# Aedelon/MASt3R-SLAM

Measured on AMD Instinct MI355X. Metric: keyframe-pairs/sec (512x512 two-view infer+match+GN), higher is better.
Workload: dtype fp16

## Files before the change

### mast3r-slam_amd/csrc/conv_tail.hip

```cpp
#include "gemm_common.h"

using namespace m3gemm;

namespace {

constexpr int kThreads = 512;
constexpr int TH = 16, TW = 32;
constexpr int HH = TH + 2, HW = TW + 2;
constexpr int kHaloPix = HH * HW;
constexpr int kHaloBytes = kHaloPix * 128;
constexpr int kWStage = 128 * 128;
constexpr int PH = 11, PW = 19;
constexpr int kPatchBytes = (PH * PW * 128 + 1023) / 1024 * 1024;
constexpr int kLdsBytes = kHaloBytes + 2 * kWStage + kPatchBytes;

struct TailArgs {
    const bf16_t *X;
    const bf16_t *Wc;
    const float *bias;
    const bf16_t *W4;
    const float *b4;
    float *pts, *conf;
    bf16_t *Y;
    const bf16_t *R;
    int cout, relu_in;
    const bf16_t *zero16;
    int B, H, W, IH, IW;
    const bf16_t *Wc2, *W42;
    const float *bias2, *b42;
};

enum { EP_PLAIN = 0 , EP_TAIL = 1 , EP_RELU = 2 ,
       EP_ADD = 3  };

template <int DT, bool UPS, int CIN, int EP>
__global__ void __launch_bounds__(kThreads, 2)
k_conv_tail(const TailArgs ain) {
    constexpr bool TAIL = EP == EP_TAIL;
    static_assert(CIN % 64 == 0 && (TAIL ? CIN == 128 : true), "64-channel steps; the fused tail is the 128-channel head.2");
    constexpr int NQ = CIN / 64;
    TailArgs a = ain;
    if (blockIdx.y == 1) {
        a.Wc = ain.Wc2; a.W4 = ain.W42; a.bias = ain.bias2; a.b4 = ain.b42;
        a.X = ain.X + (size_t)ain.B * ain.IH * ain.IW * CIN;
        if (TAIL) {
            a.pts = ain.pts + (size_t)ain.B * ain.H * ain.W * 3;
            a.conf = ain.conf + (size_t)ain.B * ain.H * ain.W;
        } else {
            a.Y = ain.Y + (size_t)ain.B * ain.H * ain.W * ain.cout;
            if (EP == EP_ADD) a.R = ain.R + (size_t)ain.B * ain.H * ain.W * ain.cout;
        }
    }
    if (!TAIL) {
        const int z = blockIdx.z;
        a.Wc += (size_t)z * 128 * 9 * CIN;
        if (a.bias) a.bias += z * 128;
        a.Y += z * 128;
        if (EP == EP_ADD) a.R += z * 128;
    }
    extern __shared__ __attribute__((aligned(16))) unsigned char lds[];
    unsigned char *halo = lds, *wst = lds + kHaloBytes, *patch = lds + kHaloBytes + 2 * kWStage;
    const int tid = threadIdx.x, lane = tid & 63, wave = tid >> 6;
    const int wp = wave >> 1, wc = wave & 1;
    const int tiles_x = (a.W + TW - 1) / TW, tiles_y = a.H / TH;
    const int nwg = tiles_x * tiles_y * a.B;
    const int bid = xcd_remap(blockIdx.x, nwg);
    const int b = bid / (tiles_x * tiles_y), trem = bid - b * tiles_x * tiles_y;
    const int ty = trem / tiles_x, tx = trem - ty * tiles_x;
    const int oy0 = ty * TH, ox0 = tx * TW;
    const bf16_t *img = a.X + (size_t)b * a.IH * a.IW * CIN;

    auto stage_w = [&](int tap, int half, int buf) {
        unsigned char *base = wst + buf * kWStage;
#pragma unroll
        for (int i = 0; i < 2; ++i) {
            const int slot = i * kThreads + tid;
            const int row = slot >> 3, cp = slot & 7;
            const int c = half * 8 + (cp ^ ((row >> 1) & 7));
            glds16(a.Wc + ((size_t)row * 9 + tap) * CIN + c * 8, base + i * (kThreads * 16) + wave * 1024);
        }
    };
    const float sy = UPS && a.H > 1 ? (float)(a.IH - 1) / (float)(a.H - 1) : 0.f;
    const float sx = UPS && a.W > 1 ? (float)(a.IW - 1) / (float)(a.W - 1) : 0.f;
    const int py0 = (int)((float)max(oy0 - 1, 0) * sy), px0 = (int)((float)max(ox0 - 1, 0) * sx);
    auto stage_patch = [&](int half) {
        for (int wi = wave; wi < (PH * PW * 8 + 63) / 64; wi += kThreads / 64) {
            int slot = wi * 64 + lane;
            slot = slot < PH * PW * 8 ? slot : PH * PW * 8 - 1;
            const int pp = slot >> 3, c = slot & 7;
            const int y = min(py0 + pp / PW, a.IH - 1), x = min(px0 + pp % PW, a.IW - 1);
            glds16(img + ((size_t)y * a.IW + x) * CIN + (half * 8 + c) * 8, patch + wi * 1024);
        }
    };
    auto stage_halo_direct = [&](int half) {
        for (int wi = wave; wi < (kHaloPix * 8 + 63) / 64; wi += kThreads / 64) {
            int slot = wi * 64 + lane;
            const bool live = slot < kHaloPix * 8;
            slot = live ? slot : kHaloPix * 8 - 1;
            const int pix = slot >> 3, cp = slot & 7;
            const int hy = pix / HW, hx = pix - hy * HW;
            const int iy = oy0 + hy - 1, ix = ox0 + hx - 1;
            const int c = half * 8 + (cp ^ ((hx >> 1) & 7));
            const bool in = iy >= 0 && iy < a.H && ix >= 0 && ix < a.W;
            const void *src = in ? (const void *)(img + ((size_t)iy * a.IW + ix) * CIN + c * 8) : (const void *)a.zero16;
            if (wi * 64 + 64 <= kHaloPix * 8) glds16(src, halo + wi * 1024);
            else if (live) *reinterpret_cast<uint4 *>(halo + (size_t)slot * 16) = *reinterpret_cast<const uint4 *>(src);
        }
    };
    auto blend_halo = [&]() {
        for (int slot = tid; slot < kHaloPix * 8; slot += kThreads) {
            const int pix = slot >> 3, cp = slot & 7;
            const int hy = pix / HW, hx = pix - hy * HW;
            const int iy = oy0 + hy - 1, ix = ox0 + hx - 1;
            const int c = cp ^ ((hx >> 1) & 7);
            uint4 o = make_uint4(0u, 0u, 0u, 0u);
            if (iy >= 0 && iy < a.H && ix >= 0 && ix < a.W) {
                const float fy = iy * sy, fx = ix * sx;
                int y0 = (int)fy, x0 = (int)fx;
                y0 = min(y0, a.IH - 1); x0 = min(x0, a.IW - 1);
                const int y1 = min(y0 + 1, a.IH - 1), x1 = min(x0 + 1, a.IW - 1);
                const float wy = fy - (float)y0, wx = fx - (float)x0;
                const unsigned char *p = patch + c * 16;
                union U { uint4 q; unsigned w[4]; } q00, q01, q10, q11, r;
                q00.q = *reinterpret_cast<const uint4 *>(p + ((y0 - py0) * PW + (x0 - px0)) * 128);
                q01.q = *reinterpret_cast<const uint4 *>(p + ((y0 - py0) * PW + (x1 - px0)) * 128);
                q10.q = *reinterpret_cast<const uint4 *>(p + ((y1 - py0) * PW + (x0 - px0)) * 128);
                q11.q = *reinterpret_cast<const uint4 *>(p + ((y1 - py0) * PW + (x1 - px0)) * 128);
#pragma unroll
                for (int k = 0; k < 4; ++k) {
                    const float tl = lo16<DT>(q00.w[k]) * (1.f - wx) + lo16<DT>(q01.w[k]) * wx;
                    const float bl = lo16<DT>(q10.w[k]) * (1.f - wx) + lo16<DT>(q11.w[k]) * wx;
                    const float th = hi16<DT>(q00.w[k]) * (1.f - wx) + hi16<DT>(q01.w[k]) * wx;
                    const float bh = hi16<DT>(q10.w[k]) * (1.f - wx) + hi16<DT>(q11.w[k]) * wx;
                    r.w[k] = pack16<DT>(tl * (1.f - wy) + bl * wy, th * (1.f - wy) + bh * wy);
                }
                o = r.q;
            }
            *reinterpret_cast<uint4 *>(halo + (size_t)slot * 16) = o;
        }
    };

    f32x4 acc[8][4];
#pragma unroll
    for (int i = 0; i < 8; ++i)
#pragma unroll
        for (int j = 0; j < 4; ++j) acc[i][j] = f32x4{0.f, 0.f, 0.f, 0.f};
    const int frow = lane & 15, fch = lane >> 4;
    int w_off[4];
#pragma unroll
    for (int j = 0; j < 4; ++j) {
        const int r = wc * 64 + j * 16 + frow;
        w_off[j] = r * 128 + ((fch ^ ((r >> 1) & 7)) << 4);
    }

    const int group = wave >> 2;
    bf16x8 af[8], wf[4];
    const int pix_of_row = (int)((0x3D9F2A40E6C851B7ULL >> (4 * frow)) & 15);
    auto col_offset = [&](int hx) { return hx * 128 + ((fch ^ ((hx >> 1) & 7)) << 4); };
    auto read_frags = [&](int g, int tap, int ks) {
        const int ky = tap / 3, kx = tap - ky * 3;
        const unsigned char *wsrc = wst + (g & 1) * kWStage;
        const int flip = ks << 6;
        const int c0 = col_offset(pix_of_row + kx) ^ flip;
        const int c1 = col_offset(16 + pix_of_row + kx) ^ flip;
        const unsigned char *rowp = halo + (wp * 4 + ky) * (HW * 128);
#pragma unroll
        for (int j = 0; j < 4; ++j) wf[j] = *reinterpret_cast<const bf16x8 *>(wsrc + (w_off[j] ^ flip));
#pragma unroll
        for (int i = 0; i < 8; ++i)
            af[i] = *reinterpret_cast<const bf16x8 *>(rowp + (i >> 1) * (HW * 128) + ((i & 1) ? c1 : c0));
        if (!TAIL && a.relu_in) {
#pragma unroll
            for (int i = 0; i < 8; ++i) af[i] = relu_frag(af[i]);
        }
    };
    auto mfma_all = [&]() {
        __builtin_amdgcn_s_setprio(1);
#pragma unroll
        for (int i = 0; i < 8; ++i)
#pragma unroll
            for (int j = 0; j < 4; ++j) acc[i][j] = mfma16<DT>(wf[j], af[i], acc[i][j]);
        __builtin_amdgcn_s_setprio(0);
    };
    auto phase_end = [&]() {
        __builtin_amdgcn_sched_barrier(0);
        __builtin_amdgcn_s_barrier();
        __builtin_amdgcn_sched_barrier(0);
    };
    auto phase_end_wait = [&]() {
        __builtin_amdgcn_sched_barrier(0);
        asm volatile("s_waitcnt vmcnt(0)" ::: "memory");
        __builtin_amdgcn_s_barrier();
        __builtin_amdgcn_sched_barrier(0);
    };
    auto prefetch_w = [&](int g) { if (g + 1 < 9 * NQ) stage_w((g + 1) % 9, (g + 1) / 9, (g + 1) & 1); };
    auto run_half = [&](int half) {
        if (group == 0) {
#pragma unroll 1
            for (int tap = 0; tap < 9; ++tap) {
                const int g = half * 9 + tap;
                read_frags(g, tap, 0);
                prefetch_w(g);
                asm volatile("s_waitcnt lgkmcnt(0)" ::: "memory");
                phase_end();
                mfma_all();
                phase_end();
                read_frags(g, tap, 1);
                asm volatile("s_waitcnt lgkmcnt(0)" ::: "memory");
                phase_end();
                mfma_all();
                phase_end_wait();
            }
            phase_end();
        } else {
#pragma unroll 1
            for (int tap = 0; tap < 9; ++tap) {
                const int g = half * 9 + tap;
                if (tap > 0) mfma_all();
                phase_end();
                read_frags(g, tap, 0);
                prefetch_w(g);
                asm volatile("s_waitcnt lgkmcnt(0)" ::: "memory");
                phase_end();
                mfma_all();
                phase_end();
                read_frags(g, tap, 1);
                asm volatile("s_waitcnt lgkmcnt(0)" ::: "memory");
                phase_end_wait();
            }
            mfma_all();
            phase_end();
        }
    };

    stage_w(0, 0, 0);
    if (UPS) stage_patch(0); else stage_halo_direct(0);
    asm volatile("s_waitcnt vmcnt(0)" ::: "memory");
    lds_barrier();
#pragma unroll 1
    for (int q = 0; q < NQ; ++q) {
        if (UPS) {
            blend_halo();
            lds_barrier();
            if (q + 1 < NQ) stage_patch(q + 1);
        } else if (q > 0) {
            stage_halo_direct(q);
            asm volatile("s_waitcnt vmcnt(0)" ::: "memory");
            lds_barrier();
        }
        run_half(q);
    }

    if constexpr (EP == EP_ADD) {
        const int r = lane & 15, gq = lane >> 4;
        constexpr int RS = 272;
        unsigned char *wl = halo + wave * (32 * RS);
        float4 bj[4];
#pragma unroll
        for (int j = 0; j < 4; ++j)
            bj[j] = a.bias ? *reinterpret_cast<const float4 *>(a.bias + wc * 64 + j * 16 + gq * 4) : make_float4(0.f, 0.f, 0.f, 0.f);
        auto pix = [&](int pass, int rl, int &oy, int &ox) {
            const int i = pass * 2 + (rl >> 4);
            oy = oy0 + wp * 4 + (i >> 1);
            ox = ox0 + (i & 1) * 16 + (int)((0x3D9F2A40E6C851B7ULL >> (4 * (rl & 15))) & 15);
        };
        uint4 q[2][4];
        auto load_resid = [&](int pass, uint4 (&dst)[4]) {
#pragma unroll
            for (int it = 0; it < 4; ++it) {
                const int c = it * 64 + lane, rl = c >> 3, ch = c & 7;
                int oy, ox;
                pix(pass, rl, oy, ox);
                ox = ox < a.W ? ox : a.W - 1;
                dst[it] = *reinterpret_cast<const uint4 *>(a.R + (((size_t)b * a.H + oy) * a.W + ox) * a.cout + wc * 64 + ch * 8);
            }
        };
        load_resid(0, q[0]);
#pragma unroll
        for (int pass = 0; pass < 4; ++pass) {
            if (pass + 1 < 4) load_resid(pass + 1, q[(pass + 1) & 1]);
#pragma unroll
            for (int ii = 0; ii < 2; ++ii)
#pragma unroll
                for (int j = 0; j < 4; ++j) {
                    const f32x4 v = acc[pass * 2 + ii][j];
                    *reinterpret_cast<float4 *>(wl + (ii * 16 + r) * RS + ((j * 4 + gq) << 4)) =
                        make_float4(v[0] + bj[j].x, v[1] + bj[j].y, v[2] + bj[j].z, v[3] + bj[j].w);
                }
            asm volatile("s_waitcnt lgkmcnt(0)" ::: "memory");
#pragma unroll
            for (int it = 0; it < 4; ++it) {
                const int c = it * 64 + lane, rl = c >> 3, ch = c & 7;
                const float4 f0 = *reinterpret_cast<const float4 *>(wl + rl * RS + ch * 32);
                const float4 f1 = *reinterpret_cast<const float4 *>(wl + rl * RS + ch * 32 + 16);
                const uint4 u = q[pass & 1][it];
                uint4 o;
                o.x = pack16<DT>(f0.x + lo16<DT>(u.x), f0.y + hi16<DT>(u.x));
                o.y = pack16<DT>(f0.z + lo16<DT>(u.y), f0.w + hi16<DT>(u.y));
                o.z = pack16<DT>(f1.x + lo16<DT>(u.z), f1.y + hi16<DT>(u.z));
                o.w = pack16<DT>(f1.z + lo16<DT>(u.w), f1.w + hi16<DT>(u.w));
                int oy, ox;
                pix(pass, rl, oy, ox);
                if (ox < a.W)
                    *reinterpret_cast<uint4 *>(a.Y + (((size_t)b * a.H + oy) * a.W + ox) * a.cout + wc * 64 + ch * 8) = o;
            }
            asm volatile("" ::: "memory");
        }
    } else if constexpr (!TAIL) {
        const int r = lane & 15, gq = lane >> 4;
        unsigned char *wl = halo + wave * 8192;
        float4 bj[4];
#pragma unroll
        for (int j = 0; j < 4; ++j)
            bj[j] = a.bias ? *reinterpret_cast<const float4 *>(a.bias + wc * 64 + j * 16 + gq * 4) : make_float4(0.f, 0.f, 0.f, 0.f);
#pragma unroll
        for (int pass = 0; pass < 2; ++pass) {
#pragma unroll
            for (int ii = 0; ii < 4; ++ii)
#pragma unroll
                for (int j = 0; j < 4; ++j) {
                    f32x4 v = acc[pass * 4 + ii][j];
                    v[0] += bj[j].x; v[1] += bj[j].y; v[2] += bj[j].z; v[3] += bj[j].w;
                    if (EP == EP_RELU) {
#pragma unroll
                        for (int e = 0; e < 4; ++e) v[e] = v[e] > 0.f ? v[e] : 0.f;
                    }
                    uint2 pk;
                    pk.x = pack16<DT>(v[0], v[1]); pk.y = pack16<DT>(v[2], v[3]);
                    *reinterpret_cast<uint2 *>(wl + (ii * 16 + r) * 128 + (((j * 2 + (gq >> 1)) ^ ((r >> 1) & 7)) << 4) + (((gq ^ r) & 1) << 3)) = pk;
                }
            asm volatile("s_waitcnt lgkmcnt(0)" ::: "memory");
#pragma unroll
            for (int it = 0; it < 8; ++it) {
                const int c = it * 64 + lane, rl = c >> 3, ch = c & 7;
                uint4 v = *reinterpret_cast<const uint4 *>(wl + rl * 128 + ((ch ^ ((rl >> 1) & 7)) << 4));
                if (rl & 1) v = uint4{v.z, v.w, v.x, v.y};
                const int i = pass * 4 + (rl >> 4);
                const int oy = oy0 + wp * 4 + (i >> 1);
                const int ox = ox0 + (i & 1) * 16 + (int)((0x3D9F2A40E6C851B7ULL >> (4 * (rl & 15))) & 15);
                if (ox < a.W)
                    *reinterpret_cast<uint4 *>(a.Y + (((size_t)b * a.H + oy) * a.W + ox) * a.cout + wc * 64 + ch * 8) = v;
            }
            asm volatile("" ::: "memory");
        }
    } else {
        const int r = lane & 15, gq = lane >> 4;
        float part[8][4];
    #pragma unroll
        for (int i = 0; i < 8; ++i)
    #pragma unroll
            for (int o = 0; o < 4; ++o) part[i][o] = 0.f;
    #pragma unroll
        for (int j = 0; j < 4; ++j) {
            const int n = wc * 64 + j * 16 + gq * 4;
            const float4 bq = a.bias ? *reinterpret_cast<const float4 *>(a.bias + n) : make_float4(0.f, 0.f, 0.f, 0.f);
            float w4[4][4];
    #pragma unroll
            for (int o = 0; o < 4; ++o) {
                const uint2 q = *reinterpret_cast<const uint2 *>(a.W4 + (size_t)o * 128 + n);
                w4[o][0] = lo16<DT>(q.x); w4[o][1] = hi16<DT>(q.x); w4[o][2] = lo16<DT>(q.y); w4[o][3] = hi16<DT>(q.y);
            }
    #pragma unroll
            for (int i = 0; i < 8; ++i) {
                const f32x4 v = acc[i][j];
                const float h[4] = {fmaxf(v[0] + bq.x, 0.f), fmaxf(v[1] + bq.y, 0.f), fmaxf(v[2] + bq.z, 0.f), fmaxf(v[3] + bq.w, 0.f)};
    #pragma unroll
                for (int o = 0; o < 4; ++o)
                    part[i][o] += (h[0] * w4[o][0] + h[1] * w4[o][1]) + (h[2] * w4[o][2] + h[3] * w4[o][3]);
            }
        }
    #pragma unroll
        for (int i = 0; i < 8; ++i)
    #pragma unroll
            for (int o = 0; o < 4; ++o) {
                float v = part[i][o];
                v += __shfl_xor(v, 16, 64);
                v += __shfl_xor(v, 32, 64);
                part[i][o] = v;
            }
        float *red = reinterpret_cast<float *>(wst);
        if (gq == 0) {
    #pragma unroll
            for (int i = 0; i < 8; ++i)
                *reinterpret_cast<float4 *>(red + (((wp * 2 + wc) * 8 + i) * 16 + r) * 4) = make_float4(part[i][0], part[i][1], part[i][2], part[i][3]);
        }
        __syncthreads();
        {
            const int i = 4 * wc + gq;
            const float4 p0 = *reinterpret_cast<const float4 *>(red + (((wp * 2 + 0) * 8 + i) * 16 + r) * 4);
            const float4 p1 = *reinterpret_cast<const float4 *>(red + (((wp * 2 + 1) * 8 + i) * 16 + r) * 4);
            const int oy = oy0 + wp * 4 + (i >> 1), ox = ox0 + (i & 1) * 16 + pix_of_row;
            if (ox < a.W) {
                const float x = p0.x + p1.x + a.b4[0], y = p0.y + p1.y + a.b4[1];
                const float z = p0.z + p1.z + a.b4[2], c = p0.w + p1.w + a.b4[3];
                const float d = sqrtf(x * x + y * y + z * z);
                const float sc = expm1f(d) / fmaxf(d, 1e-8f);
                const size_t m = ((size_t)b * a.H + oy) * a.W + ox;
                a.pts[3 * m + 0] = x * sc; a.pts[3 * m + 1] = y * sc; a.pts[3 * m + 2] = z * sc;
                a.conf[m] = 1.0f + expf(c);
            }
        }
    }
}

}

extern "C" {

static int dpt_tail_launch(const void *X, const void *Wc, const float *bias, const void *W4, const float *b4,
                           const void *Wc2, const float *bias2, const void *W42, const float *b42, float *pts,
                           float *conf, void *Y, const void *R, const void *zero16, int B, int H, int W, int cin, int cout,
                           int ep, int relu_in, int upsample, int dtype, void *stream) {
    const int groups = Wc2 ? 2 : 1;
    const bool tail = ep == EP_TAIL;
    M3_REQUIRE(X && Wc && zero16 && B > 0 && H > 0 && W > 0 && H % 16 == 0 && W % 16 == 0);
    M3_REQUIRE(tail ? (W4 && b4 && pts && conf && cin == 128 && !Y)
                    : (Y && (cin == 128 || cin == 256) && (cout == 128 || cout == 256) && (ep == EP_PLAIN || ep == EP_RELU || ep == EP_ADD)));
    M3_REQUIRE((ep == EP_ADD) == (R != nullptr) && (!upsample || ep == EP_PLAIN || tail));
    M3_REQUIRE(groups == 1 || ((!tail || (W42 && b42)) && (bias == nullptr) == (bias2 == nullptr)));
    M3_REQUIRE((dtype == DT_BF16 || dtype == DT_F16) && (!upsample || (H % 2 == 0 && W % 2 == 0)));
    M3_REQUIRE((int64_t)groups * B * H * W < (1ll << 31));
    M3_REQUIRE(reinterpret_cast<uintptr_t>(X) % 16 == 0 && reinterpret_cast<uintptr_t>(Wc) % 16 == 0 &&
               reinterpret_cast<uintptr_t>(Y) % 16 == 0 && reinterpret_cast<uintptr_t>(R) % 16 == 0);
    TailArgs a;
    a.Wc2 = (const bf16_t *)Wc2; a.W42 = (const bf16_t *)W42; a.bias2 = bias2; a.b42 = b42;
    a.X = (const bf16_t *)X; a.Wc = (const bf16_t *)Wc; a.bias = bias; a.W4 = (const bf16_t *)W4; a.b4 = b4;
    a.pts = pts; a.conf = conf; a.Y = (bf16_t *)Y; a.R = (const bf16_t *)R; a.cout = tail ? 128 : cout; a.relu_in = relu_in;
    a.zero16 = (const bf16_t *)zero16; a.B = B; a.H = H; a.W = W;
    a.IH = upsample ? H / 2 : H; a.IW = upsample ? W / 2 : W;
    const dim3 grid((unsigned)((H / TH) * ((W + TW - 1) / TW) * B), groups, tail ? 1 : cout / 128), blk(kThreads);
    hipStream_t st = (hipStream_t)stream;
#define M3_TAIL(DTV, UP, CI, EPV)                                                                                \
    do {                                                                                                         \
        static M3AttrOnce once;                                                                                  \
        int dev__;                                                                                               \
        if (m3_attr_need(once, &dev__)) {                                                                        \
            M3_CHECK_HIP(hipFuncSetAttribute(reinterpret_cast<const void *>(&k_conv_tail<DTV, UP, CI, EPV>),     \
                                             hipFuncAttributeMaxDynamicSharedMemorySize, kLdsBytes), "m3_dpt_tail/attr"); \
            m3_attr_done(once, dev__);                                                                           \
        }                                                                                                        \
        hipLaunchKernelGGL((k_conv_tail<DTV, UP, CI, EPV>), grid, blk, kLdsBytes, st, a);                        \
    } while (0)
#define M3_TAIL_DT(UP, CI, EPV) do { if (dtype == DT_F16) M3_TAIL(DT_F16, UP, CI, EPV); else M3_TAIL(DT_BF16, UP, CI, EPV); } while (0)
    if (tail) { if (upsample) M3_TAIL_DT(true, 128, EP_TAIL); else M3_TAIL_DT(false, 128, EP_TAIL); }
    else if (ep == EP_PLAIN && cin == 128) { if (upsample) M3_TAIL_DT(true, 128, EP_PLAIN); else M3_TAIL_DT(false, 128, EP_PLAIN); }
    else if (ep == EP_PLAIN) { if (upsample) M3_TAIL_DT(true, 256, EP_PLAIN); else M3_TAIL_DT(false, 256, EP_PLAIN); }
    else if (ep == EP_RELU) { if (cin == 128) M3_TAIL_DT(false, 128, EP_RELU); else M3_TAIL_DT(false, 256, EP_RELU); }
    else { if (cin == 128) M3_TAIL_DT(false, 128, EP_ADD); else M3_TAIL_DT(false, 256, EP_ADD); }
#undef M3_TAIL_DT
#undef M3_TAIL
    M3_CHECK_LAUNCH("m3_dpt_tail");
    return M3_OK;
}

int m3_dpt_tail_grouped2_dt(const void *X, const void *Wc0, const void *Wc1, const float *bias0, const float *bias1,
                            const void *W40, const void *W41, const float *b40, const float *b41, float *pts,
                            float *conf, const void *zero16, int B, int H, int W, int upsample, int dtype, void *stream) {
    M3_REQUIRE(pts && conf && (Wc1 == nullptr) == (W41 == nullptr));
    if (!Wc1) bias1 = b41 = nullptr;
    return dpt_tail_launch(X, Wc0, bias0, W40, b40, Wc1, bias1, W41, b41, pts, conf, nullptr, nullptr, zero16, B, H, W, 128, 128,
                           EP_TAIL, 0, upsample, dtype, stream);
}

int m3_conv3x3_up_direct_grouped2_dt(const void *X, const void *Wc0, const void *Wc1, const float *bias0, const float *bias1,
                                     void *Y, const void *zero16, int B, int H, int W, int Cin, int upsample, int dtype,
                                     void *stream) {
    M3_REQUIRE(Y != nullptr);
    return dpt_tail_launch(X, Wc0, bias0, nullptr, nullptr, Wc1, Wc1 ? bias1 : nullptr, nullptr, nullptr, nullptr, nullptr, Y,
                           nullptr, zero16, B, H, W, Cin, 128, EP_PLAIN, 0, upsample, dtype, stream);
}

int m3_conv3x3_direct_grouped2_dt(const void *X, const void *W0, const void *W1, const float *bias0, const float *bias1,
                                  void *Y, const void *R, const void *zero16, int B, int H, int W, int Cin, int Cout,
                                  int epilogue, int dtype, void *stream) {
    const int relu_in = (epilogue & 0x100) ? 1 : 0;
    const int e = epilogue & 0xff;
    M3_REQUIRE(Y != nullptr && (e == M3_EPI_BF16 || e == M3_EPI_BF16_RELU || e == M3_EPI_BF16_ADD));
    const int ep = e == M3_EPI_BF16 ? EP_PLAIN : (e == M3_EPI_BF16_RELU ? EP_RELU : EP_ADD);
    return dpt_tail_launch(X, W0, bias0, nullptr, nullptr, W1, bias1, nullptr, nullptr, nullptr, nullptr, Y, R, zero16, B, H, W,
                           Cin, Cout, ep, relu_in, 0, dtype, stream);
}

}
```

Baseline: 297.6.

## Overlap halo loads and upsample blending with MFMA loop via register-held slots

The direct path now loads the next channel-half halo into registers while the current half's MFMA loop runs, and applies ReLU once at store time instead of on every fragment read. The upsample path precomputes per-pixel bilinear geometry (offsets and weights) into a new LDS region. It then interleaves blending of the next half's halo slots into the tap loop and restages the patch later. This hides global-load latency and blend ALU work behind matrix math, at the cost of more registers, more LDS and a more complex schedule. Explicit fma/no-contract helpers keep the rounding of the interpolation the same as before.

```diff
diff --git a/mast3r-slam_amd/csrc/conv_tail.hip b/mast3r-slam_amd/csrc/conv_tail.hip
--- a/mast3r-slam_amd/csrc/conv_tail.hip
+++ b/mast3r-slam_amd/csrc/conv_tail.hip
@@ -12,7 +12,8 @@
 constexpr int kWStage = 128 * 128;
 constexpr int PH = 11, PW = 19;
 constexpr int kPatchBytes = (PH * PW * 128 + 1023) / 1024 * 1024;
-constexpr int kLdsBytes = kHaloBytes + 2 * kWStage + kPatchBytes;
+constexpr int kGeoBytes = kHaloPix * 16;
+constexpr int kLdsBytes = kHaloBytes + 2 * kWStage + kPatchBytes + kGeoBytes;
 
 struct TailArgs {
     const bf16_t *X;
@@ -32,6 +33,13 @@
 
 enum { EP_PLAIN = 0 , EP_TAIL = 1 , EP_RELU = 2 ,
        EP_ADD = 3  };
+
+__device__ __forceinline__ float mul_rn(float a, float b) {
+#pragma clang fp contract(off)
+    return a * b;
+}
+__device__ __forceinline__ float lerp_fuse1(float a, float b, float w1, float w) { return __builtin_fmaf(a, w1, mul_rn(b, w)); }
+__device__ __forceinline__ float lerp_fuse2(float a, float b, float w1, float w) { return __builtin_fmaf(b, w, mul_rn(a, w1)); }
 
 template <int DT, bool UPS, int CIN, int EP>
 __global__ void __launch_bounds__(kThreads, 2)
@@ -60,6 +68,7 @@
     }
     extern __shared__ __attribute__((aligned(16))) unsigned char lds[];
     unsigned char *halo = lds, *wst = lds + kHaloBytes, *patch = lds + kHaloBytes + 2 * kWStage;
+    uint4 *geo = reinterpret_cast<uint4 *>(patch + kPatchBytes);
     const int tid = threadIdx.x, lane = tid & 63, wave = tid >> 6;
     const int wp = wave >> 1, wc = wave & 1;
     const int tiles_x = (a.W + TW - 1) / TW, tiles_y = a.H / TH;
@@ -92,52 +101,70 @@
             glds16(img + ((size_t)y * a.IW + x) * CIN + (half * 8 + c) * 8, patch + wi * 1024);
         }
     };
-    auto stage_halo_direct = [&](int half) {
-        for (int wi = wave; wi < (kHaloPix * 8 + 63) / 64; wi += kThreads / 64) {
-            int slot = wi * 64 + lane;
-            const bool live = slot < kHaloPix * 8;
-            slot = live ? slot : kHaloPix * 8 - 1;
+    constexpr int kHeld = (kHaloPix * 8 + kThreads - 1) / kThreads;
+    uint4 held[kHeld];
+    auto load_held = [&](int half) {
+        int t = tid;
+        asm volatile("" : "+v"(t));
+#pragma unroll
+        for (int i = 0; i < kHeld; ++i) {
+            const int slot = min(i * kThreads + t, kHaloPix * 8 - 1);
             const int pix = slot >> 3, cp = slot & 7;
             const int hy = pix / HW, hx = pix - hy * HW;
             const int iy = oy0 + hy - 1, ix = ox0 + hx - 1;
             const int c = half * 8 + (cp ^ ((hx >> 1) & 7));
             const bool in = iy >= 0 && iy < a.H && ix >= 0 && ix < a.W;
             const void *src = in ? (const void *)(img + ((size_t)iy * a.IW + ix) * CIN + c * 8) : (const void *)a.zero16;
-            if (wi * 64 + 64 <= kHaloPix * 8) glds16(src, halo + wi * 1024);
-            else if (live) *reinterpret_cast<uint4 *>(halo + (size_t)slot * 16) = *reinterpret_cast<const uint4 *>(src);
-        }
-    };
-    auto blend_halo = [&]() {
-        for (int slot = tid; slot < kHaloPix * 8; slot += kThreads) {
-            const int pix = slot >> 3, cp = slot & 7;
+            held[i] = *reinterpret_cast<const uint4 *>(src);
+        }
+    };
+    auto store_slot = [&](int i, uint4 v) {
+        const int slot = i * kThreads + tid;
+        if ((i + 1) * kThreads <= kHaloPix * 8 || slot < kHaloPix * 8) *reinterpret_cast<uint4 *>(halo + (size_t)slot * 16) = v;
+    };
+    auto store_held = [&]() {
+        const bool relu = !TAIL && a.relu_in;
+#pragma unroll
+        for (int i = 0; i < kHeld; ++i)
+            store_slot(i, relu ? __builtin_bit_cast(uint4, relu_frag(__builtin_bit_cast(bf16x8, held[i]))) : held[i]);
+    };
+    auto build_geo = [&]() {
+        for (int pix = tid; pix < kHaloPix; pix += kThreads) {
             const int hy = pix / HW, hx = pix - hy * HW;
             const int iy = oy0 + hy - 1, ix = ox0 + hx - 1;
-            const int c = cp ^ ((hx >> 1) & 7);
-            uint4 o = make_uint4(0u, 0u, 0u, 0u);
+            uint4 g = make_uint4(1u, 0u, 0u, 0u);
             if (iy >= 0 && iy < a.H && ix >= 0 && ix < a.W) {
-                const float fy = iy * sy, fx = ix * sx;
-                int y0 = (int)fy, x0 = (int)fx;
+                int y0 = (int)mul_rn((float)iy, sy), x0 = (int)mul_rn((float)ix, sx);
                 y0 = min(y0, a.IH - 1); x0 = min(x0, a.IW - 1);
                 const int y1 = min(y0 + 1, a.IH - 1), x1 = min(x0 + 1, a.IW - 1);
-                const float wy = fy - (float)y0, wx = fx - (float)x0;
-                const unsigned char *p = patch + c * 16;
-                union U { uint4 q; unsigned w[4]; } q00, q01, q10, q11, r;
-                q00.q = *reinterpret_cast<const uint4 *>(p + ((y0 - py0) * PW + (x0 - px0)) * 128);
-                q01.q = *reinterpret_cast<const uint4 *>(p + ((y0 - py0) * PW + (x1 - px0)) * 128);
-                q10.q = *reinterpret_cast<const uint4 *>(p + ((y1 - py0) * PW + (x0 - px0)) * 128);
-                q11.q = *reinterpret_cast<const uint4 *>(p + ((y1 - py0) * PW + (x1 - px0)) * 128);
-#pragma unroll
-                for (int k = 0; k < 4; ++k) {
-                    const float tl = lo16<DT>(q00.w[k]) * (1.f - wx) + lo16<DT>(q01.w[k]) * wx;
-                    const float bl = lo16<DT>(q10.w[k]) * (1.f - wx) + lo16<DT>(q11.w[k]) * wx;
-                    const float th = hi16<DT>(q00.w[k]) * (1.f - wx) + hi16<DT>(q01.w[k]) * wx;
-                    const float bh = hi16<DT>(q10.w[k]) * (1.f - wx) + hi16<DT>(q11.w[k]) * wx;
-                    r.w[k] = pack16<DT>(tl * (1.f - wy) + bl * wy, th * (1.f - wy) + bh * wy);
-                }
-                o = r.q;
-            }
-            *reinterpret_cast<uint4 *>(halo + (size_t)slot * 16) = o;
-        }
+                const float wy = __builtin_fmaf((float)iy, sy, -(float)y0), wx = __builtin_fmaf((float)ix, sx, -(float)x0);
+                const unsigned o00 = ((y0 - py0) * PW + (x0 - px0)) * 128, o01 = ((y0 - py0) * PW + (x1 - px0)) * 128;
+                const unsigned o10 = ((y1 - py0) * PW + (x0 - px0)) * 128, o11 = ((y1 - py0) * PW + (x1 - px0)) * 128;
+                g = make_uint4(o00 | (unsigned)(((hx >> 1) & 7) << 4) | (o01 << 16), o10 | (o11 << 16), __float_as_uint(wx), __float_as_uint(wy));
+            }
+            geo[pix] = g;
+        }
+    };
+    auto blend_slot = [&](int i) {
+        const uint4 g = geo[min(i * (kThreads / 8) + (tid >> 3), kHaloPix - 1)];
+        const float wx = __uint_as_float(g.z), wy = __uint_as_float(g.w);
+        const unsigned char *p = patch + (((tid & 7) << 4) ^ (g.x & 0x70));
+        const unsigned keep = (g.x & 1) ? 0u : ~0u;
+        union U { uint4 q; unsigned w[4]; } q00, q01, q10, q11, r;
+        q00.q = *reinterpret_cast<const uint4 *>(p + (g.x & 0xff80));
+        q01.q = *reinterpret_cast<const uint4 *>(p + (g.x >> 16));
+        q10.q = *reinterpret_cast<const uint4 *>(p + (g.y & 0xffff));
+        q11.q = *reinterpret_cast<const uint4 *>(p + (g.y >> 16));
+#pragma unroll
+        for (int k = 0; k < 4; ++k) {
+            const float tl = lerp_fuse1(lo16<DT>(q00.w[k]), lo16<DT>(q01.w[k]), 1.f - wx, wx);
+            const float bl = lerp_fuse1(lo16<DT>(q10.w[k]), lo16<DT>(q11.w[k]), 1.f - wx, wx);
+            const float th = lerp_fuse2(hi16<DT>(q00.w[k]), hi16<DT>(q01.w[k]), 1.f - wx, wx);
+            const float bh = lerp_fuse2(hi16<DT>(q10.w[k]), hi16<DT>(q11.w[k]), 1.f - wx, wx);
+            r.w[k] = pack16<DT>(lerp_fuse2(tl, bl, 1.f - wy, wy), lerp_fuse1(th, bh, 1.f - wy, wy)) & keep;
+        }
+        const uint4 o = r.q;
+        return o;
     };
 
     f32x4 acc[8][4];
@@ -169,10 +196,6 @@
 #pragma unroll
         for (int i = 0; i < 8; ++i)
             af[i] = *reinterpret_cast<const bf16x8 *>(rowp + (i >> 1) * (HW * 128) + ((i & 1) ? c1 : c0));
-        if (!TAIL && a.relu_in) {
-#pragma unroll
-            for (int i = 0; i < 8; ++i) af[i] = relu_frag(af[i]);
-        }
     };
     auto mfma_all = [&]() {
         __builtin_amdgcn_s_setprio(1);
@@ -194,17 +217,30 @@
         __builtin_amdgcn_sched_barrier(0);
     };
     auto prefetch_w = [&](int g) { if (g + 1 < 9 * NQ) stage_w((g + 1) % 9, (g + 1) / 9, (g + 1) & 1); };
+    auto blend_ahead = [&](int half, int tap, int ks) {
+        if constexpr (UPS) {
+            if (tap >= 1 && tap <= kHeld / 2 && half + 1 < NQ) {
+                const uint4 v = blend_slot(2 * (tap - 1) + ks);
+#pragma unroll
+                for (int i = 0; i + 1 < kHeld; ++i) held[i] = held[i + 1];
+                held[kHeld - 1] = v;
+            }
+            if (tap == kHeld / 2 + 1 && ks == 0 && half + 2 < NQ) stage_patch(half + 2);
+        }
+    };
     auto run_half = [&](int half) {
         if (group == 0) {
 #pragma unroll 1
             for (int tap = 0; tap < 9; ++tap) {
                 const int g = half * 9 + tap;
+                blend_ahead(half, tap, 0);
                 read_frags(g, tap, 0);
                 prefetch_w(g);
                 asm volatile("s_waitcnt lgkmcnt(0)" ::: "memory");
                 phase_end();
                 mfma_all();
                 phase_end();
+                blend_ahead(half, tap, 1);
                 read_frags(g, tap, 1);
                 asm volatile("s_waitcnt lgkmcnt(0)" ::: "memory");
                 phase_end();
@@ -218,12 +254,14 @@
                 const int g = half * 9 + tap;
                 if (tap > 0) mfma_all();
                 phase_end();
+                blend_ahead(half, tap, 0);
                 read_frags(g, tap, 0);
                 prefetch_w(g);
                 asm volatile("s_waitcnt lgkmcnt(0)" ::: "memory");
                 phase_end();
                 mfma_all();
                 phase_end();
+                blend_ahead(half, tap, 1);
                 read_frags(g, tap, 1);
                 asm volatile("s_waitcnt lgkmcnt(0)" ::: "memory");
                 phase_end_wait();
@@ -234,20 +272,22 @@
     };
 
     stage_w(0, 0, 0);
-    if (UPS) stage_patch(0); else stage_halo_direct(0);
+    if (UPS) { build_geo(); stage_patch(0); } else load_held(0);
     asm volatile("s_waitcnt vmcnt(0)" ::: "memory");
-    lds_barrier();
+    if (UPS) {
+        lds_barrier();
+#pragma unroll
+        for (int i = 0; i < kHeld; ++i) {
+            store_slot(i, blend_slot(i));
+            if (i & 1) __builtin_amdgcn_sched_barrier(0);
+        }
+    }
 #pragma unroll 1
     for (int q = 0; q < NQ; ++q) {
-        if (UPS) {
-            blend_halo();
-            lds_barrier();
-            if (q + 1 < NQ) stage_patch(q + 1);
-        } else if (q > 0) {
-            stage_halo_direct(q);
-            asm volatile("s_waitcnt vmcnt(0)" ::: "memory");
-            lds_barrier();
-        }
+        if (!UPS || q > 0) store_held();
+        lds_barrier();
+        if (UPS) { if (q == 0 && NQ > 1) stage_patch(1); }
+        else if (q + 1 < NQ) load_held(q + 1);
         run_half(q);
     }
 
```

New measurement: 298.2, median of 6. About the same (+0.2%).
